# denix56/SI-Mamba

Hardware: AMD Instinct MI355X
Metric: point-clouds/sec (fwd+bwd) (higher is better)
Workload: dtype f32; 1 GPU; PointMamba classifier train step (FPS+kNN grouping, encoder, spectral SAST ordering, 12 Mamba blocks d=384 at L=1024, head, AdamW), 1024 pts -> 128 patches; global_batch=64, per_gpu_batch=64, npoints=1024, patches=128, mamba_seq_len=1024, parallelism=dp1, communicator_ranks=1, library_gemm=tuned solution table (si_mamba_amd/tuned/gemm_gfx950.csv)

## Files before the change

### include/simamba.h

```cpp
#ifndef SIMAMBA_H_
#define SIMAMBA_H_

#include <stddef.h>

#ifdef __cplusplus
extern "C" {
#endif

#define SIMAMBA_ABI_VERSION 9

#define SIMAMBA_F32  0
#define SIMAMBA_BF16 1

#define SIMAMBA_OK            0
#define SIMAMBA_E_NULLPTR    -1
#define SIMAMBA_E_SHAPE      -2
#define SIMAMBA_E_DTYPE      -3
#define SIMAMBA_E_DSTATE     -4
#define SIMAMBA_E_WIDTH      -5
#define SIMAMBA_E_WORKSPACE  -6
#define SIMAMBA_E_GROUPS     -7
#define SIMAMBA_E_ALIGN      -8
#define SIMAMBA_E_VARIANT    -9
#define SIMAMBA_E_BIAS       -10
// ... 127 lines not shown

int simamba_in_proj_fwd(const void* x, const void* w, void* xz, int batch, int L, int C, int M, int io_dtype,
                        void* stream);

int simamba_bn_relu_grid(long long rows);
int simamba_bn_relu_fwd(const void* x, const float* gterm, int group, const float* weight, const float* bias,
                        float* running_mean, float* running_var, float momentum, float eps, int training,
                        void* y, float* mean, float* invstd, float* partial, long long rows, int C,
                        long long ld, int io_dtype, void* stream);
int simamba_bn_relu_bwd(const void* dy, const void* x, const float* gterm, int group, const float* weight,
                        const float* bias, const float* mean, const float* invstd, void* dx, float* dgterm,
                        int dgroup, float* dweight, float* dbias, float* partial, long long rows, int C,
                        long long ld, int io_dtype, int training, void* stream);
int simamba_bn_stats_local(const void* x, const float* gterm, int group, double* stats, long long stats_ld,
                           float* partial, long long rows, int C, long long ld, int io_dtype, void* stream);
int simamba_bn_stats_merge(const double* stats, int world, float* running_mean, float* running_var, float momentum,
                           float eps, float* mean, float* invstd, double* count, int C, void* stream);
int simamba_bn_relu_apply(const void* x, const float* gterm, int group, const float* weight, const float* bias,
                          const float* mean, const float* invstd, void* y, long long rows, int C, long long ld,
                          int io_dtype, void* stream);
int simamba_bn_relu_bwd_sums(const void* dy, const void* x, const float* gterm, int group, const float* weight,
                             const float* bias, const float* mean, const float* invstd, float* dweight,
                             float* dbias, float* partial, long long rows, int C, long long ld, int io_dtype,
                             void* stream);
int simamba_bn_relu_bwd_dx(const void* dy, const void* x, const float* gterm, int group, const float* weight,
                           const float* bias, const float* mean, const float* invstd, const float* sum_dweight,
                           const float* sum_dbias, const double* count, void* dx, float* dgterm, int dgroup,
                           long long rows, int C, long long ld, int io_dtype, void* stream);
int simamba_group_max_fwd(const void* x, void* out, unsigned char* idx, long long groups, int n, int C,
                          int io_dtype, void* stream);
int simamba_group_max_bwd(const void* dout, const unsigned char* idx, void* dx, long long groups, int n, int C,
                          int io_dtype, void* stream);

int simamba_three_nn(const float* xyz1, const float* xyz2, int* idx, float* weight, int batch, int N, int S,
                     void* stream);
int simamba_three_interpolate_fwd(const void* feats, const int* idx, const float* weight, void* out, int batch,
                                  int N, int S, int C, int io_dtype, void* stream);
int simamba_three_interpolate_bwd(const void* dout, const int* idx, const float* weight, float* dfeats, int batch,
                                  int N, int S, int C, int io_dtype, void* stream);

int simamba_chamfer_fwd(const float* pred, const float* gt, float* dist, unsigned char* idx1, unsigned char* idx2,
                        long long pairs, int n, int m, void* stream);
int simamba_chamfer_bwd(const float* pred, const float* gt, const float* ddist, const unsigned char* idx1,
                        const unsigned char* idx2, float* dpred, long long pairs, int n, int m, void* stream);

int simamba_knn_group(const float* points, const float* centers, long long* idx, int batch, int N, int G, int K,
                      void* stream);
int simamba_knn_group_ex(const float* points, const float* centers, const long long* len_points,
                         const long long* len_centers, long long* idx, int batch, int N, int G, int K, void* stream);

#define SIMAMBA_SPEC_SYMMETRIC   0x01u
#define SIMAMBA_SPEC_SELF_LOOP   0x02u
#define SIMAMBA_SPEC_BINARY      0x04u
#define SIMAMBA_SPEC_MATRIX_SYM  0x08u
#define SIMAMBA_SPEC_SMALLEST    0x10u
#define SIMAMBA_SPEC_SIGMA_MEAN  0x20u
#define SIMAMBA_SPEC_LARGE_G     0x40u

int simamba_knn_graph(const float* points, float* adj, void* workspace, size_t ws_bytes,
                      int B, int G, int F, int knn, float alpha, unsigned flags, void* stream);

int simamba_laplacian_topk(const float* adj, float* evals, float* evecs, long long* order,
                           float* all_evals, float* all_evecs, int B, int G, int k,
                           unsigned flags, void* stream);

size_t simamba_laplacian_topk_workspace_bytes(int B, int G);
// ... 22 lines not shown
```

### si_mamba_amd/_lib.py

```python
from __future__ import annotations

import ctypes
import os
from ctypes import c_char_p, c_float, c_int, c_longlong, c_size_t, c_uint, c_void_p

_HERE = os.path.dirname(os.path.abspath(__file__))
LIB_PATH = os.path.join(_HERE, "libsimamba_hip.so")

F32, BF16 = 0, 1

SPEC_SYMMETRIC = 0x01
SPEC_SELF_LOOP = 0x02
SPEC_BINARY = 0x04
SPEC_MATRIX_SYM = 0x08
SPEC_SMALLEST = 0x10
SPEC_SIGMA_MEAN = 0x20
SPEC_LARGE_G = 0x40
SPEC_MAX_G = 128
SPEC_MAX_G_LARGE = 512

SCAN_AUTO, SCAN_ROWSCAN, SCAN_LPC2, SCAN_LPC4, SCAN_MIX = 0, 1, 2, 4, 6
CKPT_ROW, CKPT_SEQ = 128, 16
BWD_DETERMINISTIC = 1
NORM_RMS = 1
# ... 41 lines not shown
    "simamba_causal_conv1d_fwd": (c_int, [_P, _P, _P, _P, c_int, c_int, c_int, c_int, c_int, c_int, _LL, _P]),
    "simamba_causal_conv1d_bwd": (c_int, [_P, _P, _P, _P, _P, _P, _P,
                                          c_int, c_int, c_int, c_int, c_int, c_int, _LL, _LL, _P]),
    "simamba_causal_conv1d_bwd_workspace_floats": (_LL, [c_int, c_int, c_int, c_int, c_int]),
    "simamba_causal_conv1d_bwd_ex": (c_int, [_P, _P, _P, _P, _P, _P, _P,
                                             c_int, c_int, c_int, c_int, c_int, c_int, _LL, _LL, c_int, _P, _LL, _P]),
    "simamba_add_layer_norm_grid": (c_int, [c_int, c_int]),
    "simamba_add_layer_norm_fwd": (c_int, [_P, _P, _P, _P, _P, _P, _P, _P, _P, c_int, c_int, c_int, c_float,
                                           c_int, c_int, _P]),
    "simamba_add_layer_norm_bwd": (c_int, [_P, _P, _P, _P, _P, _P, _P, _P, _P, _P, c_int, c_int, c_int,
                                           c_int, c_int, _P]),
    "simamba_add_layer_norm_fwd_ex": (c_int, [_P, _P, _P, _P, _P, _P, _P, _P, _P, c_int, c_int, c_int, c_float,
                                              c_int, c_int, c_int, _P]),
    "simamba_add_layer_norm_bwd_ex": (c_int, [_P, _P, _P, _P, _P, _P, _P, _P, _P, _P, c_int, c_int, c_int,
                                              c_int, c_int, c_int, _P]),
    "simamba_out_proj_add_ln_fwd": (c_int, [_P, _P, _P, _P, _P, _P, _P, _P, _P, _P, c_int, c_int, c_int, c_int, c_float,
                                            c_int, _P]),
    "simamba_out_proj_add_ln_fwd_ex": (c_int, [_P, _P, _P, _P, _P, _P, _P, _P, _P, _P, c_int, c_int, c_int, c_int,
                                               c_float, c_int, c_int, _P]),
    "simamba_in_proj_fwd": (c_int, [_P, _P, _P, c_int, c_int, c_int, c_int, c_int, _P]),
    "simamba_bn_relu_grid": (c_int, [_LL]),
    "simamba_bn_relu_fwd": (c_int, [_P, _P, c_int, _P, _P, _P, _P, c_float, c_float, c_int, _P, _P, _P, _P, _LL, c_int,
                                    _LL, c_int, _P]),
    "simamba_bn_relu_bwd": (c_int, [_P, _P, _P, c_int, _P, _P, _P, _P, _P, _P, c_int, _P, _P, _P, _LL, c_int, _LL,
                                    c_int, c_int, _P]),
    "simamba_bn_stats_local": (c_int, [_P, _P, c_int, _P, _LL, _P, _LL, c_int, _LL, c_int, _P]),
    "simamba_bn_stats_merge": (c_int, [_P, c_int, _P, _P, c_float, c_float, _P, _P, _P, c_int, _P]),
    "simamba_bn_relu_apply": (c_int, [_P, _P, c_int, _P, _P, _P, _P, _P, _LL, c_int, _LL, c_int, _P]),
    "simamba_bn_relu_bwd_sums": (c_int, [_P, _P, _P, c_int, _P, _P, _P, _P, _P, _P, _P, _LL, c_int, _LL, c_int, _P]),
    "simamba_bn_relu_bwd_dx": (c_int, [_P, _P, _P, c_int, _P, _P, _P, _P, _P, _P, _P, _P, _P, c_int, _LL, c_int, _LL,
                                       c_int, _P]),
    "simamba_group_max_fwd": (c_int, [_P, _P, _P, _LL, c_int, c_int, c_int, _P]),
    "simamba_group_max_bwd": (c_int, [_P, _P, _P, _LL, c_int, c_int, c_int, _P]),
    "simamba_three_nn": (c_int, [_P, _P, _P, _P, c_int, c_int, c_int, _P]),
    "simamba_three_interpolate_fwd": (c_int, [_P, _P, _P, _P, c_int, c_int, c_int, c_int, c_int, _P]),
    "simamba_three_interpolate_bwd": (c_int, [_P, _P, _P, _P, c_int, c_int, c_int, c_int, c_int, _P]),
    "simamba_chamfer_fwd": (c_int, [_P, _P, _P, _P, _P, _LL, c_int, c_int, _P]),
    "simamba_chamfer_bwd": (c_int, [_P, _P, _P, _P, _P, _P, _LL, c_int, c_int, _P]),
    "simamba_knn_group": (c_int, [_P, _P, _P, c_int, c_int, c_int, c_int, _P]),
    "simamba_knn_group_ex": (c_int, [_P, _P, _P, _P, _P, c_int, c_int, c_int, c_int, _P]),
    "simamba_knn_graph": (c_int, [_P, _P, _P, c_size_t, c_int, c_int, c_int, c_int, c_float, c_uint, _P]),
    "simamba_laplacian_topk": (c_int, [_P, _P, _P, _P, _P, _P, c_int, c_int, c_int, c_uint, _P]),
    "simamba_laplacian_topk_workspace_bytes": (c_size_t, [c_int, c_int]),
    "simamba_laplacian_topk_ex": (c_int, [_P, _P, _P, _P, _P, c_size_t, c_int, c_int, c_int, c_uint, _P]),
    "simamba_spectral_workspace_bytes": (c_size_t, [c_int, c_int]),
    "simamba_spectral_topk": (c_int, [_P, _P, _P, _P, _P, c_size_t, c_int, c_int, c_int, c_float,
                                      c_int, c_uint, _P]),
    "simamba_argsort_rows": (c_int, [_P, _P, c_int, c_int, _P]),
    "simamba_farthest_point_sample": (c_int, [_P, _P, _P, c_int, c_int, c_int, _P]),
    "simamba_farthest_point_sample_ex": (c_int, [_P, _P, _P, _P, _P, c_int, c_int, c_int, _P]),
}

_lib = None


def load():
    global _lib
    if _lib is not None:
        return _lib
    if not os.path.exists(LIB_PATH):
        raise RuntimeError(
            f"{LIB_PATH} not found: build it with `python -c 'import __graft_entry__ as g; g.build()'` "
            "or `make -C si_mamba_amd/csrc`.  si_mamba_amd has no CPU / eager fallback.")
    lib = ctypes.CDLL(LIB_PATH)
    for name, (res, args) in SIGNATURES.items():
        fn = getattr(lib, name)
# ... 133 lines not shown
def spectral_large_g_forced():
    return _spectral_large_g[0]


_fuse_dt = [None]
counters = {}


def count(name):
    counters[name] = counters.get(name, 0) + 1


class scan_fuse_dt(_Override):
    cell, coerce = _fuse_dt, staticmethod(_tristate)


def fuse_dt_enabled(dtype):
    import torch
    return (dtype == torch.bfloat16) if _fuse_dt[0] is None else _fuse_dt[0]


_fuse_out_norm = [True]
_hand_in_proj = [None]


class fuse_out_norm(_Override):
    cell = _fuse_out_norm


def fuse_out_norm_enabled():
    return _fuse_out_norm[0]


class hand_in_proj(_Override):
    cell, coerce = _hand_in_proj, staticmethod(_tristate)


def in_proj_hand_enabled(workgroups, dtype=None):
    import torch
    if _hand_in_proj[0] is not None:
        return _hand_in_proj[0]
    return dtype != torch.float32 and workgroups >= IN_PROJ_MIN_WORKGROUPS


IN_PROJ_MIN_WORKGROUPS = 192


def scan_plan_step(batch, dim, seqlen, dstate, dtype, *, softplus=True, has_z=True, act_addr_or=0, a_addr=0,
                   b_addr=0, c_addr=0, z_bs=0, dz_bs=0, bc_strides=(0, 0, 0)):
    lib = load()
    code = dtype_code(dtype)
    step = _scan_ckpt[0] or lib.simamba_scan_ckpt_step(batch, dim, seqlen, dstate, code)
    if step == CKPT_SEQ and not lib.simamba_scan_seq_applicable(
            batch, dim, seqlen, dstate, code, int(bool(softplus)), int(bool(has_z)), act_addr_or, a_addr, b_addr,
            c_addr, z_bs, dz_bs, *bc_strides):
        step = CKPT_ROW
    if _scan_variant[0] == SCAN_ROWSCAN:
        step = CKPT_ROW
    return step


def mixer_scan_operands(xz_addr, a_addr, dim, seqlen, dt_rank, dstate, esz, xz_bs):
    S = dt_rank + 2 * dstate
    return dict(softplus=True, has_z=True, act_addr_or=xz_addr | (xz_addr + dim * seqlen * esz), a_addr=a_addr,
                b_addr=dt_rank * esz, c_addr=(dt_rank + dstate) * esz, z_bs=xz_bs, dz_bs=xz_bs,
                bc_strides=(seqlen * S, 1, S))
# ... 54 lines not shown
```

### si_mamba_amd/csrc/host_common.h

```cpp
#pragma once
#include "common.h"

namespace simamba {

inline int check_io_dtype(int io_dtype) {
  return (io_dtype != SIMAMBA_F32 && io_dtype != SIMAMBA_BF16) ? SIMAMBA_E_DTYPE : SIMAMBA_OK;
}
inline size_t io_esz(int io_dtype) { return io_dtype == SIMAMBA_F32 ? 4 : 2; }
inline int io_pack(int io_dtype) { return io_dtype == SIMAMBA_F32 ? 4 : 8; }
inline bool aligned16(const void* p) { return (reinterpret_cast<uintptr_t>(p) & 15u) == 0; }

template <typename F>
inline decltype(auto) with_io_type(int io_dtype, F&& f) {
  if (io_dtype == SIMAMBA_F32) return f(float{});
  return f(bf16_t{});
}

}
```

### si_mamba_amd/csrc/spectral.hip

```cpp
#include "spectral_device.h"

namespace simamba {

constexpr int kGraphThreads = 256;
constexpr int kEigThreads = 1024;

__global__ void dist_sum_kernel(const float* __restrict__ pts, double* __restrict__ acc, int G, int F) {
  __shared__ double sred[kGraphThreads];
  const float* P = pts + static_cast<size_t>(blockIdx.x) * G * F;
  double s = 0.0;
  for (int e = threadIdx.x; e < G * G; e += kGraphThreads) {
    const int i = e / G, j = e - i * G;
    s += static_cast<double>(point_dist(P, i, j, F));
  }
  sred[threadIdx.x] = s;
  __syncthreads();
  for (int w = kGraphThreads / 2; w > 0; w >>= 1) {
    if (threadIdx.x < w) sred[threadIdx.x] += sred[threadIdx.x + w];
    __syncthreads();
  }
  if (threadIdx.x == 0) atomicAdd(acc, sred[0]);
}

constexpr int kKnnLanes = 4;
// ... 299 lines not shown
constexpr int kBigTileLds = 4 * (kSpecMaxG * (kSpecMaxG + 1) + kSpecMaxG * 64 + 2 * kSpecMaxG * kKnnMaxK);

static int check_groups(int B, int G, int max_g = kSpecMaxG) {
  if (B < 0) return SIMAMBA_E_SHAPE;
  if (G < 2 || G > max_g) return SIMAMBA_E_GROUPS;
  return SIMAMBA_OK;
}

static int check_topk(int B, int G, int k, unsigned flags, int max_g, int* need) {
  const int rc = check_groups(B, G, max_g);
  if (rc) return rc;
  *need = k + ((flags & SIMAMBA_SPEC_MATRIX_SYM) ? 1 : 0);
  if (k < 0 || *need > G) return SIMAMBA_E_GROUPS;
  return SIMAMBA_OK;
}

extern "C" int simamba_knn_graph(const float* points, float* adj, void* workspace, size_t ws_bytes, int B, int G,
                                 int F, int knn, float alpha, unsigned flags, void* stream) {
  if (!points || !adj) return SIMAMBA_E_NULLPTR;
  int rc = check_groups(B, G, kSpecMaxGLarge);
  if (rc) return rc;
  if (F < 1 || F > 64 || knn < 0 || knn + 1 > G || knn + 1 > kKnnMaxK) return SIMAMBA_E_GROUPS;
  if (B == 0) return SIMAMBA_OK;
  hipStream_t s = static_cast<hipStream_t>(stream);
  double* acc = nullptr;
  if (flags & SIMAMBA_SPEC_SIGMA_MEAN) {
    if (!workspace || ws_bytes < 256) return SIMAMBA_E_WORKSPACE;
    acc = static_cast<double*>(workspace);
    hipError_t e = hipMemsetAsync(acc, 0, sizeof(double), s);
    if (e != hipSuccess) return static_cast<int>(e);
    hipLaunchKernelGGL(dist_sum_kernel, dim3(B), dim3(kGraphThreads), 0, s, points, acc, G, F);
  }
  if (G > kSpecMaxG) return launch_knn_graph_large(points, adj, acc, B, G, F, knn, alpha, flags, s);
  ensure_lds_cap<knn_graph_kernel>(kBigTileLds);
  const size_t smem = sizeof(float) * (static_cast<size_t>(G) * (G + 1) + G * F + 2 * G * kKnnMaxK);
  hipLaunchKernelGGL(knn_graph_kernel, dim3(B), dim3(G * kKnnLanes), smem, s, points, adj, acc, B, G, F, knn, alpha,
                     flags);
  return static_cast<int>(hipGetLastError());
}

extern "C" int simamba_laplacian_topk(const float* adj, float* evals, float* evecs, long long* order,
                                      float* all_evals, float* all_evecs, int B, int G, int k, unsigned flags,
                                      void* stream) {
  if (!adj) return SIMAMBA_E_NULLPTR;
  int need;
  const int rc = check_topk(B, G, k, flags, kSpecMaxG, &need);
  if (rc) return rc;
  if (B == 0) return SIMAMBA_OK;
  EigArgs a{adj, evals, evecs, order, all_evals, all_evecs, B, G, k, flags};
  if (!all_evals && !all_evecs && need <= kTdMaxSel && G >= 3)
    return launch_tridiag_topk(a, static_cast<hipStream_t>(stream));
  const size_t smem = sizeof(float) * kSpecMaxG * kEigLD;
  ensure_lds_cap<laplacian_eig_kernel>(kBigTileLds);
  hipLaunchKernelGGL(laplacian_eig_kernel, dim3(B), dim3(kEigThreads), smem, static_cast<hipStream_t>(stream), a);
  return static_cast<int>(hipGetLastError());
}

constexpr unsigned kSpecKnownFlags = SIMAMBA_SPEC_SYMMETRIC | SIMAMBA_SPEC_SELF_LOOP | SIMAMBA_SPEC_BINARY |
                                     SIMAMBA_SPEC_MATRIX_SYM | SIMAMBA_SPEC_SMALLEST | SIMAMBA_SPEC_SIGMA_MEAN |
                                     SIMAMBA_SPEC_LARGE_G;

extern "C" int simamba_laplacian_topk_ex(const float* adj, float* evals, float* evecs, long long* order,
                                         void* workspace, size_t ws_bytes, int B, int G, int k, unsigned flags,
                                         void* stream) {
  if (!adj) return SIMAMBA_E_NULLPTR;
  if (flags & ~kSpecKnownFlags) return SIMAMBA_E_VARIANT;
  int need;
  const int rc = check_topk(B, G, k, flags, kSpecMaxGLarge, &need);
  if (rc) return rc;
  const bool large = G > kSpecMaxG || (flags & SIMAMBA_SPEC_LARGE_G);
  if (!large)
    return simamba_laplacian_topk(adj, evals, evecs, order, nullptr, nullptr, B, G, k, flags, stream);
  if (need > kTdMaxSel) return SIMAMBA_E_GROUPS;
  if (!workspace) return SIMAMBA_E_NULLPTR;
  if (ws_bytes < simamba_laplacian_topk_workspace_bytes(B, G)) return SIMAMBA_E_WORKSPACE;
  if (B == 0) return SIMAMBA_OK;
  EigArgs a{adj, evals, evecs, order, nullptr, nullptr, B, G, k, flags};
  return launch_laplacian_large_topk(a, static_cast<float*>(workspace), static_cast<hipStream_t>(stream));
}

extern "C" int simamba_spectral_topk(const float* centers, float* evals, float* evecs, long long* order,
                                     void* workspace, size_t ws_bytes, int B, int G, int knn, float alpha, int k,
                                     unsigned flags, void* stream) {
  if (!centers || !workspace) return SIMAMBA_E_NULLPTR;
  if (ws_bytes < simamba_spectral_workspace_bytes(B, G)) return SIMAMBA_E_WORKSPACE;
  float* adj = reinterpret_cast<float*>(static_cast<char*>(workspace) + 256);
// ... 18 lines not shown
```

### si_mamba_amd/csrc/spectral_common.h

```cpp
#pragma once
#include "common.h"

namespace simamba {

constexpr int kSpecMaxG = 128;
constexpr int kSpecMaxGLarge = 512;
constexpr int kKnnMaxK = 32;
constexpr int kTdMaxSel = 8;

struct EigArgs {
  const float* adj;
  float* evals;
  float* evecs;
  long long* order;
  float* all_evals;
  float* all_evecs;
  int B, G, k;
  unsigned flags;
};

template <auto kKernel>
inline void ensure_lds_cap(int bytes) {
  static const bool once = [bytes] {
    (void)hipFuncSetAttribute(reinterpret_cast<const void*>(kKernel), hipFuncAttributeMaxDynamicSharedMemorySize,
                              bytes);
    return true;
  }();
  (void)once;
}

int launch_tridiag_topk(const EigArgs& a, hipStream_t s);
int launch_knn_graph_large(const float* pts, float* adj, const double* dist_sum, int B, int G, int F, int knn,
                           float alpha, unsigned flags, hipStream_t s);
int launch_laplacian_large_topk(const EigArgs& a, float* ws, hipStream_t s);

}
```

### si_mamba_amd/csrc/spectral_large.hip

```cpp
#include "spectral_device.h"


namespace simamba {

__device__ __forceinline__ void global_barrier() {
  __builtin_amdgcn_s_waitcnt(0x0F70);
  __syncthreads();
}

constexpr int kKnnRows = 128;
constexpr int kKnnRowLanes = 8;
constexpr int kKnnRowThreads = kKnnRows * kKnnRowLanes;

template <bool kMirror>
__global__ __launch_bounds__(kKnnRowThreads) void knn_rows_kernel(const float* __restrict__ pts,
                                                                  float* __restrict__ adj,
                                                                  const double* __restrict__ dist_sum, int B, int G,
                                                                  int F, int knn, float alpha, unsigned flags) {
  extern __shared__ float sP[];
  const int tid = threadIdx.x;
  const float* P = pts + static_cast<size_t>(blockIdx.x) * G * F;
  float* A = adj + static_cast<size_t>(blockIdx.x) * G * G;
  const int r0 = blockIdx.y * kKnnRows;
  const int nrows = min(kKnnRows, G - r0);
// ... 7 lines not shown
  if (i >= G) return;
  float pv = -1.f;
  int pi = -1;
  for (int m = 0; m <= knn; ++m) {
    float bv = 3.0e38f;
    int bi = 0x7fffffff;
    for (int j = part; j < G; j += kKnnRowLanes) {
      const float v = point_dist(sP, i, j, F);
      const bool after_prev = (v > pv) || (v == pv && j > pi);
      if (after_prev && (v < bv)) { bv = v; bi = j; }
    }
#pragma unroll
    for (int off = 1; off < kKnnRowLanes; off <<= 1) {
      const float ov = __shfl_xor(bv, off);
      const int oi = __shfl_xor(bi, off);
      const bool take = knn_take(ov, oi, bv, bi);
      bv = take ? ov : bv;
      bi = take ? oi : bi;
    }
    pv = bv; pi = bi;
    if (bi == 0x7fffffff) break;
    if (m == 0 && !self_loop) continue;
    const float w = knn_edge_weight(flags, bv, alpha, inv2s2);
    if (part == 0) {
      if (kMirror) A[static_cast<size_t>(bi) * G + i] = w;
      else A[static_cast<size_t>(i) * G + bi] = w;
    }
  }
}

int launch_knn_graph_large(const float* pts, float* adj, const double* dist_sum, int B, int G, int F, int knn,
                           float alpha, unsigned flags, hipStream_t s) {
  const int cap = static_cast<int>(sizeof(float)) * kSpecMaxGLarge * 64;
  ensure_lds_cap<knn_rows_kernel<false>>(cap);
  ensure_lds_cap<knn_rows_kernel<true>>(cap);
  const dim3 grid(B, (G + kKnnRows - 1) / kKnnRows);
  const size_t smem = sizeof(float) * static_cast<size_t>(G) * F;
  hipLaunchKernelGGL(knn_rows_kernel<false>, grid, dim3(kKnnRowThreads), smem, s, pts, adj, dist_sum, B, G, F, knn,
                     alpha, flags);
  if (flags & SIMAMBA_SPEC_SYMMETRIC)
    hipLaunchKernelGGL(knn_rows_kernel<true>, grid, dim3(kKnnRowThreads), smem, s, pts, adj, dist_sum, B, G, F, knn,
                       alpha, flags);
  return static_cast<int>(hipGetLastError());
}

constexpr int kLgThreads = 1024;
constexpr int kLgWaves = kLgThreads / 64;
constexpr int kLgGroups = kLgThreads / 16;
constexpr int kLgVecBatch = 4;
constexpr int kLgBtPer = kSpecMaxGLarge / 64;
constexpr size_t kLgDynLds = sizeof(double) * (kTdMaxSel + 4 * kLgVecBatch) * kSpecMaxGLarge +
                             kLgVecBatch * kSpecMaxGLarge;

__device__ __forceinline__ float lg_wave_sum_f32(float v) {
#pragma unroll
  for (int off = 32; off > 0; off >>= 1) v += __shfl_xor(v, off);
  return v;
}

__global__ __launch_bounds__(kLgThreads) void laplacian_large_kernel(EigArgs p, float* __restrict__ ws) {
  extern __shared__ __attribute__((aligned(16))) double dsm[];
  constexpr int NG = kSpecMaxGLarge;
  double* sZ = dsm;
  double* sLa = sZ + kTdMaxSel * NG;
  double* sLb = sLa + kLgVecBatch * NG;
  double* sLc = sLb + kLgVecBatch * NG;
  double* sLl = sLc + kLgVecBatch * NG;
  unsigned char* sPiv = reinterpret_cast<unsigned char*>(sLl + kLgVecBatch * NG);
// ... 156 lines not shown
        v[q] = (i == 0) ? 1.f : (i < m ? S[k * G + k + 1 + i] : 0.f);
      }
    };
    if (G >= 3) load_refl(G - 3, vn);
    for (int k = G - 3; k >= 0; --k) {
      float vk[kLgBtPer];
#pragma unroll
      for (int q = 0; q < kLgBtPer; ++q) vk[q] = vn[q];
      if (k > 0) load_refl(k - 1, vn);
      const double tau = sTau[k];
      if (tau == 0.0) continue;
      const int m = G - k - 1;
      double dot = 0.0;
#pragma unroll
      for (int q = 0; q < kLgBtPer; ++q) {
        const int i = lane + 64 * q;
        if (i < m) dot += static_cast<double>(vk[q]) * z[k + 1 + i];
      }
      dot = wave_sum_f64(dot) * tau;
#pragma unroll
      for (int q = 0; q < kLgBtPer; ++q) {
        const int i = lane + 64 * q;
        if (i < m) z[k + 1 + i] -= dot * static_cast<double>(vk[q]);
      }
    }
    sign_of_largest(z, G, lane, &sSign[sv]);
  }
  __syncthreads();

  write_topk_outputs<kLgThreads, NG>(p, sZ, sLam, sSign, skip);
}

int launch_laplacian_large_topk(const EigArgs& a, float* ws, hipStream_t s) {
  ensure_lds_cap<laplacian_large_kernel>(static_cast<int>(kLgDynLds));
  hipLaunchKernelGGL(laplacian_large_kernel, dim3(a.B), dim3(kLgThreads), kLgDynLds, s, a, ws);
  return static_cast<int>(hipGetLastError());
}

}
```

### si_mamba_amd/csrc/spectral_tridiag.hip

```cpp
#include "spectral_device.h"


namespace simamba {

constexpr int kTdThreads = 512;
constexpr int kTdGroups = kTdThreads / 16;
constexpr int kTdLD = kSpecMaxG + 1;

__device__ __forceinline__ void colnorm_partials(const float* S, int LD, int G, int col, float* sPart) {
  const int lane16 = threadIdx.x & 15, grp = threadIdx.x >> 4;
  if (lane16 == 0) {
    float acc = 0.f;
    for (int r = col + 1 + grp; r < G; r += kTdGroups) {
      const float x = S[r * LD + col];
      acc = fmaf(x, x, acc);
    }
    sPart[grp] = acc;
  }
}

__device__ __forceinline__ float sum_partials(const float* sPart) {
  float acc = 0.f;
#pragma unroll
  for (int q = 0; q < kTdGroups / 4; ++q) {
// ... 110 lines not shown
  }
  __syncthreads();
  if (lane == 0 && wave < ntot)
    tridiag_inverse_iteration(G, sLam[wave], tnorm, inverse_iteration_seed(wave), sD, sE, sLa[wave], sLb[wave],
                              sLc[wave], sLl[wave], sPiv[wave], sZ[wave]);
  __syncthreads();
  if (tid < 64) gram_schmidt_wave0<kSpecMaxG>(&sZ[0][0], ntot, G, tid);
  __syncthreads();
  for (int s = wave; s < ntot; s += kTdThreads / 64) {
    double* z = sZ[s];
    for (int k = G - 3; k >= 0; --k) {
      const double tau = sTau[k];
      if (tau == 0.0) continue;
      const int m = G - k - 1;
      double dot = 0.0;
      for (int i = lane; i < m; i += 64) {
        const double vi = (i == 0) ? 1.0 : static_cast<double>(S[(k + 1 + i) * LD + k]);
        dot += vi * z[k + 1 + i];
      }
      dot = wave_sum_f64(dot) * tau;
      for (int i = lane; i < m; i += 64) {
        const double vi = (i == 0) ? 1.0 : static_cast<double>(S[(k + 1 + i) * LD + k]);
        z[k + 1 + i] -= dot * vi;
      }
    }
    sign_of_largest(z, G, lane, &sSign[s]);
  }
  __syncthreads();

  write_topk_outputs<kTdThreads, kSpecMaxG>(p, &sZ[0][0], sLam, sSign, skip);
}

int launch_tridiag_topk(const EigArgs& a, hipStream_t s) {
  ensure_lds_cap<laplacian_tridiag_kernel>(kSpecMaxG * kTdLD * 4);
  hipLaunchKernelGGL(laplacian_tridiag_kernel, dim3(a.B), dim3(kTdThreads), sizeof(float) * kSpecMaxG * kTdLD, s, a);
  return static_cast<int>(hipGetLastError());
}

}
```

### si_mamba_amd/encoder_ops.py

```python
from __future__ import annotations

import torch
import torch.distributed as dist

from . import _lib


_BN_MAX_C = 1024
_BN_CHUNK = 256


_SPLITK = 64
_SPLITK_MIN_ROWS = 512


class TokenLinearFn(torch.autograd.Function):

    @staticmethod
    def forward(ctx, x, weight, bias):
        y = torch.nn.functional.linear(x, weight, bias)
        ctx.save_for_backward(x, weight)
        ctx.has_bias = bias is not None
        return y

# ... 274 lines not shown


class GroupMaxFn(torch.autograd.Function):
    @staticmethod
    def forward(ctx, x):
        _lib.require_gpu(x, "group_max_fn")
        xc = x.contiguous()
        groups, n, C = xc.shape
        dev = xc.device
        code = _lib.dtype_code(xc.dtype)
        out = torch.empty(groups, C, device=dev, dtype=xc.dtype)
        idx = torch.empty(groups, C, device=dev, dtype=torch.uint8)
        with torch.cuda.device(dev):
            _abi("simamba_group_max_fwd", xc.data_ptr(), out.data_ptr(), idx.data_ptr(), groups, n, C, code,
                 _lib.stream_ptr(dev))
        ctx.save_for_backward(idx)
        ctx.meta = (groups, n, C, code, xc.dtype)
        return out

    @staticmethod
    def backward(ctx, dout):
        (idx,) = ctx.saved_tensors
        groups, n, C, code, dtype = ctx.meta
        d = dout.to(dtype).contiguous()
        dx = torch.empty(groups, n, C, device=d.device, dtype=dtype)
        with torch.cuda.device(d.device):
            _abi("simamba_group_max_bwd", d.data_ptr(), idx.data_ptr(), dx.data_ptr(), groups, n, C, code,
                 _lib.stream_ptr(d.device))
        return dx


def group_max_fn(x):
    return GroupMaxFn.apply(x)
```

### si_mamba_amd/point_mamba.py

```python
from __future__ import annotations

from types import SimpleNamespace

import torch
import torch.nn as nn

from . import grouping, spectral
from .block import MixerModel
from .add_norm import add_layer_norm_fn
from .encoder_ops import bn_relu_fn, group_max_fn, token_linear


class Group(nn.Module):

    def __init__(self, num_group, group_size):
        super().__init__()
        self.num_group = num_group
        self.group_size = group_size
        self.fps_fn = grouping.sample_farthest_points

    @torch.no_grad()
    def _indices(self, xyz, lengths=None):
        if lengths is not None:
            if not (xyz.is_cuda and xyz.shape[1] <= 8192):
                raise NotImplementedError("Group: lengths are taken by the HIP kernels only (a ROCm device, clouds of "
                                          "up to 8192 points)")
            need = max(self.num_group, self.group_size)
            if not torch.cuda.is_current_stream_capturing():
                shortest = int(lengths.min())
                if shortest < need:
                    raise ValueError(f"Group: the shortest cloud has {shortest} points, every cloud needs at least "
                                     f"{need} (max of num_group = {self.num_group} and group_size = {self.group_size})")
            center, _ = self.fps_fn(xyz, self.num_group, lengths=lengths)
            return center, grouping.knn_group(center, xyz, self.group_size, lengths=lengths)
        center, _ = self.fps_fn(xyz, self.num_group)
        if xyz.is_cuda and xyz.shape[1] <= 8192:
            return center, grouping.knn_group(center, xyz, self.group_size)
        d = torch.cdist(center, xyz)
        nn_idx = d.topk(self.group_size, dim=-1, largest=False, sorted=False)[1]
        return center, nn_idx

    def forward(self, xyz, *, lengths=None):
        B, N, _ = xyz.shape
        center, nn_idx = self._indices(xyz, lengths)
        flat = (nn_idx + torch.arange(B, device=xyz.device).view(-1, 1, 1) * N).view(-1)
        nb = xyz.reshape(B * N, -1)[flat].view(B, self.num_group, self.group_size, 3).contiguous()
        return nb - center.unsqueeze(2), center, nb


class Encoder(nn.Module):

    def __init__(self, encoder_channel):
        super().__init__()
        self.encoder_channel = encoder_channel
        self.fused = True
        self.first_conv = nn.Sequential(nn.Conv1d(3, 128, 1), nn.BatchNorm1d(128), nn.ReLU(inplace=True),
                                        nn.Conv1d(128, 256, 1))
        self.second_conv = nn.Sequential(nn.Conv1d(512, 512, 1), nn.BatchNorm1d(512), nn.ReLU(inplace=True),
                                         nn.Conv1d(512, self.encoder_channel, 1))

    def forward(self, point_groups):
        bs, g, n, _ = point_groups.shape
        c1, bn1, _, c2 = self.first_conv
        c3, bn2, _, c4 = self.second_conv
        lin = torch.nn.functional.linear
        x = point_groups.reshape(bs * g * n, 3)
        if self.fused and x.is_cuda and 256 % n == 0:
            lin = token_linear
            x = bn_relu_fn(lin(x, c1.weight.squeeze(-1), c1.bias), bn1)
            f = lin(x, c2.weight.squeeze(-1), c2.bias)
            cf = f.shape[1]
            fg = group_max_fn(f.view(bs * g, n, cf))
            w3 = c3.weight.squeeze(-1)
            gterm = lin(fg, w3[:, :cf], c3.bias)
            x = bn_relu_fn(lin(f, w3[:, cf:]), bn2, gterm=gterm, group=n)
            f = lin(x, c4.weight.squeeze(-1), c4.bias)
            return group_max_fn(f.view(bs * g, n, self.encoder_channel)).reshape(bs, g, self.encoder_channel)
        x = torch.relu(bn1(lin(x, c1.weight.squeeze(-1), c1.bias)))
        f = lin(x, c2.weight.squeeze(-1), c2.bias).view(bs * g, n, 256)
        fg = f.max(dim=1, keepdim=True)[0]
        x = torch.cat([fg.expand(-1, n, -1), f], dim=2).reshape(bs * g * n, 512)
        x = torch.relu(bn2(lin(x, c3.weight.squeeze(-1), c3.bias)))
        f = lin(x, c4.weight.squeeze(-1), c4.bias).view(bs * g, n, self.encoder_channel)
        return f.max(dim=1)[0].reshape(bs, g, self.encoder_channel)


def default_config(**over):
    cfg = dict(trans_dim=384, depth=12, cls_dim=15, group_size=32, num_group=128, encoder_dims=384,
               rms_norm=False, drop_path=0.1, drop_out=0., method="SAST", reverse=True, knn_graph=20,
               k_top_eigenvectors=4, alpha=10., smallest=True, symmetric=True, self_loop=False,
               binary=True, matrix="laplacian")
    cfg.update(over)
    return SimpleNamespace(**cfg)


def plackett_luce_dist(logits):
    return torch.sum(logits - torch.logcumsumexp(logits.flip(-1), dim=-1).flip(-1), dim=-1)


class PointMamba(nn.Module):
    def __init__(self, config, **kwargs):
        super().__init__()
        self.config = config
        self.trans_dim = config.trans_dim
        self.depth = config.depth
        self.cls_dim = config.cls_dim
        self.group_size = config.group_size
        self.num_group = config.num_group
        self.encoder_dims = config.encoder_dims
        self.group_divider = Group(num_group=self.num_group, group_size=self.group_size)
# ... 124 lines not shown
```

Measured before the change: 1110 point-clouds/s.

## Add sparse backward for final encoder linear followed by group max

Fuses the last encoder linear layer with its group-max reduction and adds custom backward kernels. Only the argmax row of each group receives gradient, so dx and dW are computed sparsely from the saved indices instead of by dense GEMMs over the scattered gradient. The linear output is no longer saved for backward. In exchange it adds two bespoke kernels, one with a per-slab partial buffer and a deterministic reduction, and the bias-gradient and fallback paths add complexity. It also moves ensure_lds_cap into a shared header and makes it return an error code.

```diff
diff --git a/include/simamba.h b/include/simamba.h
--- a/include/simamba.h
+++ b/include/simamba.h
@@ -183,6 +183,12 @@
 int simamba_group_max_bwd(const void* dout, const unsigned char* idx, void* dx, long long groups, int n, int C,
                           int io_dtype, void* stream);
 
+int simamba_max_linear_bwd_slabs(long long groups, int c_in);
+int simamba_max_linear_bwd_dx(const void* dout, const unsigned char* idx, const void* weight, void* dx,
+                              long long groups, int n, int c_in, int c_out, int io_dtype, void* stream);
+int simamba_max_linear_bwd_dw(const void* dout, const unsigned char* idx, const void* x, float* dw, float* partial,
+                              long long groups, int n, int c_in, int c_out, int io_dtype, void* stream);
+
 int simamba_three_nn(const float* xyz1, const float* xyz2, int* idx, float* weight, int batch, int N, int S,
                      void* stream);
 int simamba_three_interpolate_fwd(const void* feats, const int* idx, const float* weight, void* out, int batch,
diff --git a/si_mamba_amd/_lib.py b/si_mamba_amd/_lib.py
--- a/si_mamba_amd/_lib.py
+++ b/si_mamba_amd/_lib.py
@@ -97,6 +97,9 @@
                                        c_int, _P]),
     "simamba_group_max_fwd": (c_int, [_P, _P, _P, _LL, c_int, c_int, c_int, _P]),
     "simamba_group_max_bwd": (c_int, [_P, _P, _P, _LL, c_int, c_int, c_int, _P]),
+    "simamba_max_linear_bwd_slabs": (c_int, [_LL, c_int]),
+    "simamba_max_linear_bwd_dx": (c_int, [_P, _P, _P, _P, _LL, c_int, c_int, c_int, c_int, _P]),
+    "simamba_max_linear_bwd_dw": (c_int, [_P, _P, _P, _P, _P, _LL, c_int, c_int, c_int, c_int, _P]),
     "simamba_three_nn": (c_int, [_P, _P, _P, _P, c_int, c_int, c_int, _P]),
     "simamba_three_interpolate_fwd": (c_int, [_P, _P, _P, _P, c_int, c_int, c_int, c_int, c_int, _P]),
     "simamba_three_interpolate_bwd": (c_int, [_P, _P, _P, _P, c_int, c_int, c_int, c_int, c_int, _P]),
@@ -296,6 +299,18 @@
     return _fuse_out_norm[0]
 
 
+_sparse_max_linear = [None]
+
+
+class sparse_max_linear(_Override):
+    cell, coerce = _sparse_max_linear, staticmethod(_tristate)
+
+
+def sparse_max_linear_enabled(dtype):
+    import torch
+    return (dtype == torch.float32) if _sparse_max_linear[0] is None else _sparse_max_linear[0]
+
+
 class hand_in_proj(_Override):
     cell, coerce = _hand_in_proj, staticmethod(_tristate)
 
diff --git a/si_mamba_amd/csrc/encoder_sparse.hip b/si_mamba_amd/csrc/encoder_sparse.hip
--- /dev/null
+++ b/si_mamba_amd/csrc/encoder_sparse.hip
@@ -0,0 +1,219 @@
+#include "det_reduce.h"
+#include "host_common.h"
+
+namespace simamba {
+
+constexpr int kSpCols = 64;
+constexpr int kSpWaves = 16;
+constexpr int kSpThreads = kSpWaves * 64;
+constexpr int kSpMaxN = 32;
+constexpr int kSpMaxCout = 384;
+constexpr int kSpChunks = kSpMaxCout / 64;
+constexpr int kSpCpw = kSpMaxCout / kSpWaves;
+constexpr int kSpTilePatches = 8;
+constexpr int kSpTileRegs = kSpCpw / 8;
+constexpr int kSpTileQuads = kSpTilePatches * kSpMaxN * (kSpCols / 4) / kSpThreads;
+constexpr int kSpTargetWorkgroups = 256;
+constexpr long long kSpMaxGroups = 1ll << 30;
+constexpr int kSpDxMinSlab = kSpWaves;
+static_assert(kSpTilePatches * 8 == 64 && kSpCpw % 8 == 0, "a register holds 8 channels of each of a tile's 8 patches");
+
+template <typename T>
+__device__ __forceinline__ float4 load_quad(const T* p) {
+  const Pack<T, 4> pk = *reinterpret_cast<const Pack<T, 4>*>(p);
+  return make_float4(to_f32<T>(pk.v[0]), to_f32<T>(pk.v[1]), to_f32<T>(pk.v[2]), to_f32<T>(pk.v[3]));
+}
+
+__device__ __forceinline__ float read_lane(float v, int lane) {
+  return __builtin_bit_cast(float, __builtin_amdgcn_readlane(__builtin_bit_cast(int, v), lane));
+}
+
+template <typename T>
+__global__ __launch_bounds__(kSpThreads) void max_linear_bwd_dx_kernel(
+    const T* __restrict__ dout, const unsigned char* __restrict__ idx, const T* __restrict__ W, T* __restrict__ dx,
+    long long groups, int n, int cin, int cout, int slab) {
+  extern __shared__ __attribute__((aligned(16))) float sW[];
+  const int col0 = blockIdx.x * kSpCols;
+  const int lane = threadIdx.x & 63;
+  const int wave = __builtin_amdgcn_readfirstlane(threadIdx.x >> 6);
+  for (int e = threadIdx.x; e < cout * (kSpCols / 4); e += kSpThreads) {
+    const int c = e / (kSpCols / 4), q = e % (kSpCols / 4);
+    *reinterpret_cast<float4*>(sW + c * kSpCols + 4 * q) = load_quad<T>(W + static_cast<long long>(c) * cin + col0 + 4 * q);
+  }
+  __syncthreads();
+  const float* wl = sW + lane;
+  const long long g0 = static_cast<long long>(blockIdx.y) * slab;
+  const long long g1 = min(g0 + slab, groups);
+  for (long long g = g0 + wave; g < g1; g += kSpWaves) {
+    int id[kSpChunks];
+    float d[kSpChunks];
+#pragma unroll
+    for (int k = 0; k < kSpChunks; ++k) {
+      const int c = 64 * k + lane;
+      const bool ok = c < cout;
+      id[k] = ok ? static_cast<int>(idx[g * cout + c]) : 255;
+      d[k] = ok ? to_f32<T>(dout[g * cout + c]) : 0.f;
+    }
+    T* out = dx + g * n * cin + col0 + lane;
+    for (int r = 0; r < n; ++r) {
+      float acc = 0.f;
+#pragma unroll
+      for (int k = 0; k < kSpChunks; ++k) {
+        unsigned long long m = __ballot(id[k] == r);
+        while (m) {
+          const int j = __builtin_ctzll(m);
+          m &= m - 1;
+          acc = fmaf(read_lane(d[k], j), wl[(64 * k + j) * kSpCols], acc);
+        }
+      }
+      out[static_cast<long long>(r) * cin] = from_f32<T>(acc);
+    }
+  }
+}
+
+template <typename T>
+__global__ __launch_bounds__(kSpThreads) void max_linear_bwd_dw_kernel(
+    const T* __restrict__ dout, const unsigned char* __restrict__ idx, const T* __restrict__ X,
+    float* __restrict__ partial, long long groups, int n, int cin, int cout, int slab) {
+  extern __shared__ __attribute__((aligned(16))) float sX[];
+  const int col0 = blockIdx.x * kSpCols;
+  const int lane = threadIdx.x & 63;
+  const int wave = __builtin_amdgcn_readfirstlane(threadIdx.x >> 6);
+  const int cpw = (cout + kSpWaves - 1) / kSpWaves;
+  const int c0 = wave * cpw;
+  const int cnt = max(0, min(cpw, cout - c0));
+  const int tile_rows = kSpTilePatches * n;
+  const long long g0 = static_cast<long long>(blockIdx.y) * slab;
+  const long long g1 = min(g0 + slab, groups);
+
+  float acc[kSpCpw];
+#pragma unroll
+  for (int j = 0; j < kSpCpw; ++j) acc[j] = 0.f;
+
+  float4 xq[kSpTileQuads];
+  int id[kSpTileRegs];
+  float d[kSpTileRegs];
+  auto fetch = [&](long long g) {
+    const long long rows = min(static_cast<long long>(kSpTilePatches), g1 - g) * n;
+#pragma unroll
+    for (int q = 0; q < kSpTileQuads; ++q) {
+      const int e = q * kSpThreads + threadIdx.x;
+      const int row = e / (kSpCols / 4), quad = e % (kSpCols / 4);
+      xq[q] = make_float4(0.f, 0.f, 0.f, 0.f);
+      if (row < rows) xq[q] = load_quad<T>(X + (g * n + row) * cin + col0 + 4 * quad);
+    }
+#pragma unroll
+    for (int q = 0; q < kSpTileRegs; ++q) {
+      const int p = lane / 8, j = q * 8 + lane % 8;
+      const bool ok = j < cnt && g + p < g1;
+      const long long at = (g + p) * cout + c0 + j;
+      const int r = ok ? static_cast<int>(idx[at]) : n;
+      id[q] = r < n ? p * n + r : tile_rows;
+      d[q] = r < n ? to_f32<T>(dout[at]) : 0.f;
+    }
+  };
+
+  if (threadIdx.x < 2 * kSpCols)
+    sX[(threadIdx.x / kSpCols) * (tile_rows + 1) * kSpCols + tile_rows * kSpCols + threadIdx.x % kSpCols] = 0.f;
+  int buf = 0;
+  if (g0 < g1) fetch(g0);
+  for (long long g = g0; g < g1; g += kSpTilePatches) {
+    float* tile = sX + buf * (tile_rows + 1) * kSpCols;
+#pragma unroll
+    for (int q = 0; q < kSpTileQuads; ++q) {
+      const int e = q * kSpThreads + threadIdx.x;
+      if (e < tile_rows * (kSpCols / 4)) *reinterpret_cast<float4*>(tile + 4 * e) = xq[q];
+    }
+    int idc[kSpTileRegs];
+    float dc[kSpTileRegs];
+#pragma unroll
+    for (int q = 0; q < kSpTileRegs; ++q) { idc[q] = id[q]; dc[q] = d[q]; }
+    __syncthreads();
+    if (g + kSpTilePatches < g1) fetch(g + kSpTilePatches);
+    const float* xl = tile + lane;
+#pragma unroll 1
+    for (int p = 0; p < kSpTilePatches; ++p) {
+#pragma unroll
+      for (int j = 0; j < kSpCpw; ++j) {
+        const int row = __builtin_amdgcn_readlane(idc[j / 8], p * 8 + j % 8);
+        acc[j] = fmaf(read_lane(dc[j / 8], p * 8 + j % 8), xl[row * kSpCols], acc[j]);
+      }
+    }
+    buf ^= 1;
+  }
+  float* out = partial + (static_cast<long long>(blockIdx.y) * cout + c0) * cin + col0 + lane;
+#pragma unroll
+  for (int j = 0; j < kSpCpw; ++j)
+    if (j < cnt) out[static_cast<long long>(j) * cin] = acc[j];
+}
+
+constexpr int kSpDxLds = kSpMaxCout * kSpCols * 4;
+constexpr int kSpDwLds = 2 * (kSpTilePatches * kSpMaxN + 1) * kSpCols * 4;
+
+static int max_linear_check(int io_dtype, long long groups, int n, int cin, int cout, bool pointers, bool aligned) {
+  if (const int rc = check_io_dtype(io_dtype)) return rc;
+  if (groups == 0) return 1;
+  if (groups < 0 || groups > kSpMaxGroups || n < 1 || n > kSpMaxN || cin < kSpCols || (cin % kSpCols) != 0 ||
+      cin > 65536 || cout < 4 || (cout % 4) != 0 || cout > kSpMaxCout)
+    return SIMAMBA_E_SHAPE;
+  if (!pointers) return SIMAMBA_E_NULLPTR;
+  if (!aligned) return SIMAMBA_E_ALIGN;
+  return SIMAMBA_OK;
+}
+
+static int slab_of(long long groups, int cin, int floor) {
+  const long long slabs = max(1ll, static_cast<long long>(kSpTargetWorkgroups / (cin / kSpCols)));
+  return static_cast<int>(max(static_cast<long long>(floor), (groups + slabs - 1) / slabs));
+}
+
+}
+
+using namespace simamba;
+
+extern "C" int simamba_max_linear_bwd_slabs(long long groups, int c_in) {
+  if (groups <= 0 || c_in < kSpCols || (c_in % kSpCols) != 0) return 0;
+  const int slab = slab_of(groups, c_in, kSpTilePatches);
+  return static_cast<int>((groups + slab - 1) / slab);
+}
+
+extern "C" int simamba_max_linear_bwd_dx(const void* dout, const unsigned char* idx, const void* weight, void* dx,
+                                         long long groups, int n, int c_in, int c_out, int io_dtype, void* stream) {
+  if (const int rc = max_linear_check(io_dtype, groups, n, c_in, c_out, dout && idx && weight && dx,
+                                      aligned16(dout) && aligned16(weight) && aligned16(dx)))
+    return rc > 0 ? SIMAMBA_OK : rc;
+  const int slab = slab_of(groups, c_in, kSpDxMinSlab);
+  const dim3 grid(c_in / kSpCols, static_cast<unsigned>((groups + slab - 1) / slab));
+  const size_t lds = sizeof(float) * c_out * kSpCols;
+  return with_io_type(io_dtype, [&](auto tag) {
+    using T = decltype(tag);
+    if (const hipError_t e = ensure_lds_cap<max_linear_bwd_dx_kernel<T>>(kSpDxLds)) return static_cast<int>(e);
+    hipLaunchKernelGGL(max_linear_bwd_dx_kernel<T>, grid, dim3(kSpThreads), lds, static_cast<hipStream_t>(stream),
+                       static_cast<const T*>(dout), idx, static_cast<const T*>(weight), static_cast<T*>(dx), groups, n,
+                       c_in, c_out, slab);
+    return static_cast<int>(hipGetLastError());
+  });
+}
+
+extern "C" int simamba_max_linear_bwd_dw(const void* dout, const unsigned char* idx, const void* x, float* dw,
+                                         float* partial, long long groups, int n, int c_in, int c_out, int io_dtype,
+                                         void* stream) {
+  if (const int rc = max_linear_check(io_dtype, groups, n, c_in, c_out, dout && idx && x && dw && partial,
+                                      aligned16(dout) && aligned16(x) && aligned16(dw) && aligned16(partial)))
+    return rc > 0 ? SIMAMBA_OK : rc;
+  hipStream_t s = static_cast<hipStream_t>(stream);
+  const int slab = slab_of(groups, c_in, kSpTilePatches);
+  const int slabs = static_cast<int>((groups + slab - 1) / slab);
+  const dim3 grid(c_in / kSpCols, slabs);
+  const size_t lds = sizeof(float) * 2 * (kSpTilePatches * n + 1) * kSpCols;
+  const int rc = with_io_type(io_dtype, [&](auto tag) {
+    using T = decltype(tag);
+    if (const hipError_t e = ensure_lds_cap<max_linear_bwd_dw_kernel<T>>(kSpDwLds)) return static_cast<int>(e);
+    hipLaunchKernelGGL(max_linear_bwd_dw_kernel<T>, grid, dim3(kSpThreads), lds, s, static_cast<const T*>(dout), idx,
+                       static_cast<const T*>(x), partial, groups, n, c_in, c_out, slab);
+    return static_cast<int>(hipGetLastError());
+  });
+  if (rc) return rc;
+  const long long elems = static_cast<long long>(c_out) * c_in;
+  const DetSumJob job{partial, dw, elems, elems, slabs};
+  return det_sum_launch(&job, 1, s);
+}
diff --git a/si_mamba_amd/csrc/host_common.h b/si_mamba_amd/csrc/host_common.h
--- a/si_mamba_amd/csrc/host_common.h
+++ b/si_mamba_amd/csrc/host_common.h
@@ -1,4 +1,6 @@
 #pragma once
+#include <atomic>
+
 #include "common.h"
 
 namespace simamba {
@@ -16,4 +18,17 @@
   return f(bf16_t{});
 }
 
+template <auto kKernel>
+inline hipError_t ensure_lds_cap(int bytes) {
+  static std::atomic<unsigned long long> done{0};
+  int dev = 0;
+  if (const hipError_t e = hipGetDevice(&dev)) return e;
+  const unsigned long long bit = (dev >= 0 && dev < 64) ? 1ull << dev : 0;
+  if (bit && (done.load(std::memory_order_acquire) & bit)) return hipSuccess;
+  const hipError_t e = hipFuncSetAttribute(reinterpret_cast<const void*>(kKernel),
+                                           hipFuncAttributeMaxDynamicSharedMemorySize, bytes);
+  if (e == hipSuccess) done.fetch_or(bit, std::memory_order_release);
+  return e;
 }
+
+}
diff --git a/si_mamba_amd/csrc/spectral.hip b/si_mamba_amd/csrc/spectral.hip
--- a/si_mamba_amd/csrc/spectral.hip
+++ b/si_mamba_amd/csrc/spectral.hip
@@ -355,7 +355,7 @@
     hipLaunchKernelGGL(dist_sum_kernel, dim3(B), dim3(kGraphThreads), 0, s, points, acc, G, F);
   }
   if (G > kSpecMaxG) return launch_knn_graph_large(points, adj, acc, B, G, F, knn, alpha, flags, s);
-  ensure_lds_cap<knn_graph_kernel>(kBigTileLds);
+  (void)ensure_lds_cap<knn_graph_kernel>(kBigTileLds);
   const size_t smem = sizeof(float) * (static_cast<size_t>(G) * (G + 1) + G * F + 2 * G * kKnnMaxK);
   hipLaunchKernelGGL(knn_graph_kernel, dim3(B), dim3(G * kKnnLanes), smem, s, points, adj, acc, B, G, F, knn, alpha,
                      flags);
@@ -374,7 +374,7 @@
   if (!all_evals && !all_evecs && need <= kTdMaxSel && G >= 3)
     return launch_tridiag_topk(a, static_cast<hipStream_t>(stream));
   const size_t smem = sizeof(float) * kSpecMaxG * kEigLD;
-  ensure_lds_cap<laplacian_eig_kernel>(kBigTileLds);
+  (void)ensure_lds_cap<laplacian_eig_kernel>(kBigTileLds);
   hipLaunchKernelGGL(laplacian_eig_kernel, dim3(B), dim3(kEigThreads), smem, static_cast<hipStream_t>(stream), a);
   return static_cast<int>(hipGetLastError());
 }
diff --git a/si_mamba_amd/csrc/spectral_common.h b/si_mamba_amd/csrc/spectral_common.h
--- a/si_mamba_amd/csrc/spectral_common.h
+++ b/si_mamba_amd/csrc/spectral_common.h
@@ -1,5 +1,5 @@
 #pragma once
-#include "common.h"
+#include "host_common.h"
 
 namespace simamba {
 
@@ -19,16 +19,6 @@
   unsigned flags;
 };
 
-template <auto kKernel>
-inline void ensure_lds_cap(int bytes) {
-  static const bool once = [bytes] {
-    (void)hipFuncSetAttribute(reinterpret_cast<const void*>(kKernel), hipFuncAttributeMaxDynamicSharedMemorySize,
-                              bytes);
-    return true;
-  }();
-  (void)once;
-}
-
 int launch_tridiag_topk(const EigArgs& a, hipStream_t s);
 int launch_knn_graph_large(const float* pts, float* adj, const double* dist_sum, int B, int G, int F, int knn,
                            float alpha, unsigned flags, hipStream_t s);
diff --git a/si_mamba_amd/csrc/spectral_large.hip b/si_mamba_amd/csrc/spectral_large.hip
--- a/si_mamba_amd/csrc/spectral_large.hip
+++ b/si_mamba_amd/csrc/spectral_large.hip
@@ -63,8 +63,8 @@
 int launch_knn_graph_large(const float* pts, float* adj, const double* dist_sum, int B, int G, int F, int knn,
                            float alpha, unsigned flags, hipStream_t s) {
   const int cap = static_cast<int>(sizeof(float)) * kSpecMaxGLarge * 64;
-  ensure_lds_cap<knn_rows_kernel<false>>(cap);
-  ensure_lds_cap<knn_rows_kernel<true>>(cap);
+  (void)ensure_lds_cap<knn_rows_kernel<false>>(cap);
+  (void)ensure_lds_cap<knn_rows_kernel<true>>(cap);
   const dim3 grid(B, (G + kKnnRows - 1) / kKnnRows);
   const size_t smem = sizeof(float) * static_cast<size_t>(G) * F;
   hipLaunchKernelGGL(knn_rows_kernel<false>, grid, dim3(kKnnRowThreads), smem, s, pts, adj, dist_sum, B, G, F, knn,
@@ -287,7 +287,7 @@
 }
 
 int launch_laplacian_large_topk(const EigArgs& a, float* ws, hipStream_t s) {
-  ensure_lds_cap<laplacian_large_kernel>(static_cast<int>(kLgDynLds));
+  (void)ensure_lds_cap<laplacian_large_kernel>(static_cast<int>(kLgDynLds));
   hipLaunchKernelGGL(laplacian_large_kernel, dim3(a.B), dim3(kLgThreads), kLgDynLds, s, a, ws);
   return static_cast<int>(hipGetLastError());
 }
diff --git a/si_mamba_amd/csrc/spectral_tridiag.hip b/si_mamba_amd/csrc/spectral_tridiag.hip
--- a/si_mamba_amd/csrc/spectral_tridiag.hip
+++ b/si_mamba_amd/csrc/spectral_tridiag.hip
@@ -166,7 +166,7 @@
 }
 
 int launch_tridiag_topk(const EigArgs& a, hipStream_t s) {
-  ensure_lds_cap<laplacian_tridiag_kernel>(kSpecMaxG * kTdLD * 4);
+  (void)ensure_lds_cap<laplacian_tridiag_kernel>(kSpecMaxG * kTdLD * 4);
   hipLaunchKernelGGL(laplacian_tridiag_kernel, dim3(a.B), dim3(kTdThreads), sizeof(float) * kSpecMaxG * kTdLD, s, a);
   return static_cast<int>(hipGetLastError());
 }
diff --git a/si_mamba_amd/encoder_ops.py b/si_mamba_amd/encoder_ops.py
--- a/si_mamba_amd/encoder_ops.py
+++ b/si_mamba_amd/encoder_ops.py
@@ -330,3 +330,78 @@
 
 def group_max_fn(x):
     return GroupMaxFn.apply(x)
+
+
+_SPARSE_MAX_N = 32
+_SPARSE_MAX_COUT = 384
+
+
+def _linear_io_dtype(x):
+    return torch.get_autocast_dtype("cuda") if (x.is_cuda and torch.is_autocast_enabled("cuda")) else x.dtype
+
+
+def token_linear_group_max_ok(x, weight, n):
+    if not (x.is_cuda and x.dim() == 2 and weight.dim() == 2 and _lib.sparse_max_linear_enabled(_linear_io_dtype(x))):
+        return False
+    rows, cin = x.shape
+    cout = weight.shape[0]
+    return (1 <= n <= _SPARSE_MAX_N and rows > 0 and rows % n == 0 and cin == weight.shape[1] and cin % 64 == 0
+            and cout % 4 == 0 and 4 <= cout <= _SPARSE_MAX_COUT
+            and _linear_io_dtype(x) in (torch.float32, torch.bfloat16)
+            and x.is_contiguous() and x.data_ptr() % 16 == 0)
+
+
+class TokenLinearGroupMaxFn(torch.autograd.Function):
+
+    @staticmethod
+    def forward(ctx, x, weight, bias, n):
+        y = torch.nn.functional.linear(x, weight, bias).contiguous()
+        rows, cout = y.shape
+        groups = rows // n
+        dev = y.device
+        code = _lib.dtype_code(y.dtype)
+        out = torch.empty(groups, cout, device=dev, dtype=y.dtype)
+        idx = torch.empty(groups, cout, device=dev, dtype=torch.uint8)
+        with torch.cuda.device(dev):
+            _abi("simamba_group_max_fwd", y.data_ptr(), out.data_ptr(), idx.data_ptr(), groups, n, cout, code,
+                 _lib.stream_ptr(dev))
+        ctx.save_for_backward(x, weight, idx)
+        ctx.meta = (groups, int(n), code, y.dtype, bias is not None)
+        return out
+
+    @staticmethod
+    def backward(ctx, dout):
+        x, weight, idx = ctx.saved_tensors
+        groups, n, code, io, has_bias = ctx.meta
+        cout, cin = weight.shape
+        dev = dout.device
+        d = dout.to(io).contiguous()
+        dx = dw = db = None
+        with torch.cuda.device(dev):
+            st = _lib.stream_ptr(dev)
+            if ctx.needs_input_grad[0]:
+                w = weight.detach().to(io).contiguous()
+                dx = torch.empty(groups * n, cin, device=dev, dtype=io)
+                _abi("simamba_max_linear_bwd_dx", d.data_ptr(), idx.data_ptr(), w.data_ptr(), dx.data_ptr(), groups, n,
+                     cin, cout, code, st)
+                dx = dx.to(x.dtype)
+            if ctx.needs_input_grad[1]:
+                xc = x.detach().to(io).contiguous()
+                slabs = _lib.load().simamba_max_linear_bwd_slabs(groups, cin)
+                part = torch.empty(slabs, cout, cin, device=dev, dtype=torch.float32)
+                dw = torch.empty(cout, cin, device=dev, dtype=torch.float32)
+                _abi("simamba_max_linear_bwd_dw", d.data_ptr(), idx.data_ptr(), xc.data_ptr(), dw.data_ptr(),
+                     part.data_ptr(), groups, n, cin, cout, code, st)
+                dw = dw.to(weight.dtype)
+        if has_bias and ctx.needs_input_grad[2]:
+            db = d.sum(0, dtype=torch.float32).to(weight.dtype)
+        return dx, dw, db, None
+
+
+def token_linear_group_max(x, weight, bias, n):
+    if token_linear_group_max_ok(x, weight, n):
+        _lib.count("max_linear_sparse")
+        return TokenLinearGroupMaxFn.apply(x, weight, bias, n)
+    _lib.count("max_linear_dense")
+    y = token_linear(x, weight, bias)
+    return group_max_fn(y.view(y.shape[0] // n, n, y.shape[1]))
diff --git a/si_mamba_amd/point_mamba.py b/si_mamba_amd/point_mamba.py
--- a/si_mamba_amd/point_mamba.py
+++ b/si_mamba_amd/point_mamba.py
@@ -8,7 +8,7 @@
 from . import grouping, spectral
 from .block import MixerModel
 from .add_norm import add_layer_norm_fn
-from .encoder_ops import bn_relu_fn, group_max_fn, token_linear
+from .encoder_ops import bn_relu_fn, group_max_fn, token_linear, token_linear_group_max
 
 
 class Group(nn.Module):
@@ -74,8 +74,7 @@
             w3 = c3.weight.squeeze(-1)
             gterm = lin(fg, w3[:, :cf], c3.bias)
             x = bn_relu_fn(lin(f, w3[:, cf:]), bn2, gterm=gterm, group=n)
-            f = lin(x, c4.weight.squeeze(-1), c4.bias)
-            return group_max_fn(f.view(bs * g, n, self.encoder_channel)).reshape(bs, g, self.encoder_channel)
+            return token_linear_group_max(x, c4.weight.squeeze(-1), c4.bias, n).reshape(bs, g, self.encoder_channel)
         x = torch.relu(bn1(lin(x, c1.weight.squeeze(-1), c1.bias)))
         f = lin(x, c2.weight.squeeze(-1), c2.bias).view(bs * g, n, 256)
         fg = f.max(dim=1, keepdim=True)[0]
```

New measurement: 1125 point-clouds/s (median of 6 runs). +1.4%, better.
